# metalcycling/polynomial_reduction_with_full_domain_decomposition_preconditioner

Hardware: AMD Instinct MI355X
Metric: PCG DOF-updates/sec + SpMV GB/s (%HBM peak), 3D Poisson N=7 (higher is better)
Workload: dtype f64; 1 GPU; 3D Poisson, 32x32x32 elements (32^3 per GPU), N=7, flexible PCG + FDD preconditioner (single subdomain = whole domain, inner GMRES(4), polynomial reduction 6); outer=fcg, mesh=box, poly_degree=7, points_per_gpu=16777216, unique_nodes=11390625, preconditioner=fdd_gmres4, comm=single

## Files before the change

include/fdd_hip.h:

```cpp
#ifndef FDD_HIP_H
#define FDD_HIP_H

#include <stddef.h>

#ifdef __cplusplus
extern "C" {
#endif

#define FDD_ERR_INVALID_ARGUMENT (-1)
#define FDD_ERR_UNSUPPORTED (-2)
#define FDD_ERR_NOT_INITIALIZED (-3)

#define FDD_NUM_GEOM_FACTS 6
#define FDD_REDUCE_MAX_BLOCKS 2048

const char *fdd_version(void);
const char *fdd_last_error(void);
int fdd_device_count(int *count);
int fdd_set_device(int device);
int fdd_get_device(int *device);
int fdd_device_name(char *buf, size_t buf_len);
int fdd_malloc(void **ptr, size_t bytes);
int fdd_free(void *ptr);
int fdd_memcpy_h2d(void *dst, const void *src, size_t bytes, void *stream);
// ... 37 lines not shown

int fdd_dom_stiffness_matrix_1(double *const GDu[3], const double *u, const double *D_hat, const double *const G[FDD_NUM_GEOM_FACTS], int num_points, int poly_degree, int dim, void *stream);
int fdd_dom_stiffness_matrix_2(double *Au, const double *const GDu[3], const double *D_hat, int num_points, int poly_degree, int dim, void *stream);
int fdd_dom_stiffness_matrix(double *Au, const double *u, const double *D_hat, const double *const G[FDD_NUM_GEOM_FACTS], int num_elements, int poly_degree, void *stream);

int fdd_stiffness_matrix_mfma(double *Au, const double *u, const double *D_hat, const double *const G[FDD_NUM_GEOM_FACTS], const int *elem_offset, int num_elements, int poly_degree, void *stream);
int fdd_stiffness_matrix_mfma_gather(double *Au, const double *v, const double *v_scale_dev, const int *point_dof, const double *D_hat, const double *const G[FDD_NUM_GEOM_FACTS], const int *elem_offset, int num_elements, int poly_degree, void *stream);
int fdd_stiffness_matrix_mfma_diag(double *Au, const double *v, const double *v_scale_dev, const int *point_dof, const double *D_hat, const double *const G[FDD_NUM_GEOM_FACTS], const int *elem_offset, int num_elements, int poly_degree, void *stream);

int fdd_dom_initialize_arrays(double *u_k, double *r_k, const double *f, int num_points, void *stream);

size_t fdd_reduce_workspace_doubles(void);
int fdd_dom_residual_norm(double *out, double *ws, const double *r_k, const double *QQt_r_k, const double *dirichlet_mask, int num_points, void *stream);
int fdd_dom_projection_inner_products(double *out2, double *ws, const double *z_k, const double *r_k, const double *p_k, const double *q_k, int num_points, void *stream);
int fdd_dom_inner_product_flexible(double *out, double *ws, const double *r_k, const double *r_kp1, const double *z_k, int num_points, void *stream);
int fdd_dom_inner_product_flexible_gamma(double *out2, double *ws, const double *r_k, const double *r_kp1, const double *z_k, int num_points, void *stream);
int fdd_dom_lincomb_flexible_gamma(double *out2, double *ws, const double *r_k, const double *r_kp1, double *z_k, int num_points, int slice_begin, int slice_size, int z_is_zero, const double *coeffs_dev, const double *const *v, const double *v_scale_dev, const double *last_dev, int m, void *stream);
int fdd_dom_inner_product(double *out, double *ws, const double *u_k, const double *v_k, const double *dirichlet_mask, int num_points, void *stream);

int fdd_dom_solution_and_residual_update(double *u_k, double *r_kp1, const double *r_k, const double *p_k, const double *q_k, double alpha_k, int num_points, void *stream);
int fdd_dom_residual_and_search_update(double *p_k, double *r_k, const double *z_k, const double *r_kp1, double beta_k, int num_points, void *stream);
int fdd_dom_solution_and_residual_update_dev(double *u_k, double *r_kp1, const double *r_k, const double *p_k, const double *q_k, const double *alpha_num, const double *alpha_den, int num_points, void *stream);
int fdd_dom_residual_and_search_update_dev(double *p_k, double *r_k, const double *z_k, const double *r_kp1, const double *beta_num, const double *beta_den, int num_points, void *stream);

int fdd_sub_stiffness_matrix_1(double *const GDu[3], const double *u, const double *const *D_hat_ptr, const int *offset, const int *vert, const int *level, const int *poly_degree, int num_levels, const double *const G[FDD_NUM_GEOM_FACTS], int num_points, int dim, void *stream);
int fdd_sub_stiffness_matrix_2(double *Au, const double *const GDu[3], const double *const *D_hat_ptr, const int *offset, const int *vert, const int *level, const int *poly_degree, int num_levels, int num_points, int dim, void *stream);
int fdd_sub_stiffness_matrix(double *Au, const double *u, const double *D_hat, const double *const G[FDD_NUM_GEOM_FACTS], const int *elem_offset, int num_elements, int poly_degree, void *stream);
int fdd_stiffness_matrix_2d(double *Au, const double *u, const double *D_hat, const double *const G[FDD_NUM_GEOM_FACTS], const int *elem_offset, int num_elements, int poly_degree, void *stream);
int fdd_sub_stiffness_matrix_gather(double *Au, const double *v, const int *point_dof, const double *D_hat, const double *const G[FDD_NUM_GEOM_FACTS], const int *elem_offset, int num_elements, int poly_degree, void *stream);

int fdd_sub_inner_product(double *out, double *ws, const double *u, const double *v, int num_values, void *stream);
int fdd_sub_weighted_inner_product(double *out, double *ws, const double *u, const double *v, const double *w, int num_values, void *stream);
int fdd_sub_projection_inner_products(double *out2, double *ws, const double *z_k, const double *r_k, const double *p_k, const double *q_k, const double *weight, int num_values, void *stream);
int fdd_sub_search_update_inner_product(double *out, double *ws, const double *r_k, const double *r_kp1, const double *z_k, const double *weight, int num_points, void *stream);
int fdd_sub_initialize_arrays(double *u_k, double *r_k, const double *f, int num_values, void *stream);
int fdd_sub_solution_and_residual_update(double *u_k, double *r_kp1, const double *r_k, const double *p_k, const double *q_k, double alpha_k, int num_values, void *stream);
int fdd_sub_residual_and_search_update(double *p_k, double *r_k, const double *z_k, const double *r_kp1, double beta_k, int num_values, void *stream);
int fdd_sub_copy_f64_f64(double *u, const double *v, int num_points, void *stream);
int fdd_sub_copy_f32_f64(float *u, const double *v, int num_points, void *stream);
int fdd_sub_copy_f64_f32(double *u, const float *v, int num_points, void *stream);
int fdd_sub_restriction_1(double *Ju, const double *J_cf, const double *u, int num_points, int n_f, int n_c, int dim, void *stream);
int fdd_sub_restriction_2(double *Ju, const double *J_cf, const double *u, int num_points, int n_f, int n_c, int dim, void *stream);
int fdd_sub_restriction_3(double *Ju, const double *J_cf, const double *u, int num_points, int n_f, int n_c, void *stream);
int fdd_sub_restriction(double *u_c, const double *J_cf, const double *u_f, int num_elements, int n_f, int n_c, void *stream);
int fdd_sub_restriction_2d(double *u_c, const double *J_cf, const double *u_f, int num_elements, int n_f, int n_c, void *stream);

// ... 139 lines not shown
```

polynomial_reduction_with_full_domain_decomposition_preconditioner_amd/csrc/fdd_blas1.hip:

```cpp
#include "fdd_stream.h"

namespace
{

constexpr int kBlock = 256;
using Single = fdd_lanes<1>;
using Pair = fdd_lanes<2>;

template <typename Op>
__global__ __launch_bounds__(kBlock) void ew_vec2_kernel(Op op, long long n2, long long n)
{
    const long long stride = (long long)gridDim.x * kBlock;
    for (long long i = (long long)blockIdx.x * kBlock + threadIdx.x; i < n2; i += stride) op.at(Pair{}, i);
    if ((n & 1) && blockIdx.x == 0 && threadIdx.x == 0) op.at(Single{}, n - 1);
}

template <typename Op>
__global__ __launch_bounds__(kBlock) void ew_scalar_kernel(Op op, long long n)
{
    const long long stride = (long long)gridDim.x * kBlock;
    for (long long i = (long long)blockIdx.x * kBlock + threadIdx.x; i < n; i += stride) op.at(Single{}, i);
}

constexpr int kEwMaxBlocks = 32768;
// ... 85 lines not shown
    }
    template <typename F>
    void pointers(F f) const { f(z), f(u), f(d); }
};

struct XpbyRatioDevOp
{
    double *out;
    const double *x, *y, *num, *den;
    template <typename A>
    __device__ void at(A a, long long i) const { a.st(out, i, a.ld(x, i) + (*num / *den) * a.ld(y, i)); }
    template <typename F>
    void pointers(F f) const { f(out), f(x), f(y); }
};

struct XmayRatioDevOp
{
    double *out;
    const double *x, *y, *num, *den;
    template <typename A>
    __device__ void at(A a, long long i) const { a.st(out, i, a.ld(x, i) - (*num / *den) * a.ld(y, i)); }
    template <typename F>
    void pointers(F f) const { f(out), f(x), f(y); }
};

struct ChebyStepOp
{
    double *x, *d, *r_out;
    const double *r_in, *q, *dinv;
    double c_d, c_r;
    int first, last;
    template <typename A>
    __device__ void at(A a, long long i) const { fdd_cheby_step_at(a, i, x, d, r_out, r_in, q, dinv, c_d, c_r, first, last); }
    template <typename F>
    void pointers(F f) const
    {
        f(x), f(r_in), f(dinv);
        if (!last) f(d);
        if (!first) f(q), f(d);
        if (!first && !last) f(r_out);
    }
};

}
__global__ void fdd_sqrt_sum_kernel(double *out, const double *parts, int nparts)
{
// ... 344 lines not shown
{
    FDD_REQUIRE(out != nullptr && parts_dev != nullptr && nparts >= 1);
    hipLaunchKernelGGL(fdd_sqrt_sum_kernel, dim3(1), dim3(64), 0, fdd_stream(stream), out, parts_dev, nparts);
    FDD_LAUNCH_CHECK();
    return 0;
}

int fdd_xpby_ratio_dev(double *out, const double *x, const double *num_dev, const double *den_dev, const double *y, int n, void *stream)
{
    FDD_REQUIRE(n >= 0);
    if (n == 0) return 0;
    FDD_REQUIRE(out != nullptr && x != nullptr && y != nullptr && num_dev != nullptr && den_dev != nullptr);
    return launch_ew(XpbyRatioDevOp{out, x, y, num_dev, den_dev}, n, stream);
}

int fdd_xmay_ratio_dev(double *out, const double *x, const double *num_dev, const double *den_dev, const double *y, int n, void *stream)
{
    FDD_REQUIRE(n >= 0);
    if (n == 0) return 0;
    FDD_REQUIRE(out != nullptr && x != nullptr && y != nullptr && num_dev != nullptr && den_dev != nullptr);
    return launch_ew(XmayRatioDevOp{out, x, y, num_dev, den_dev}, n, stream);
}

int fdd_vector_scaling_dev(double *au, const double *scale_dev, const double *u, int n, void *stream)
{
    FDD_REQUIRE(n >= 0);
    if (n == 0) return 0;
    FDD_REQUIRE(au != nullptr && u != nullptr && scale_dev != nullptr);
    return launch_ew(ScaleDevOp{au, u, scale_dev}, n, stream);
}

int fdd_vector_diagonal_scaling_dev(double *z, const double *d, const double *scale_dev, const double *u, int n, void *stream)
{
    FDD_REQUIRE(n >= 0);
    if (n == 0) return 0;
    FDD_REQUIRE(z != nullptr && u != nullptr && d != nullptr);
    return launch_ew(DiagScaleDevOp{z, d, u, scale_dev}, n, stream);
}

int fdd_cheby_step(double *x, double *d, double *r_out, const double *r_in, const double *q, const double *dinv, double c_d, double c_r, int first, int last, int n, void *stream)
{
    FDD_REQUIRE(n >= 0);
    if (n == 0) return 0;
    FDD_REQUIRE(x != nullptr && r_in != nullptr && dinv != nullptr);
    FDD_REQUIRE(last || d != nullptr);
    FDD_REQUIRE(first || (q != nullptr && d != nullptr && (last || r_out != nullptr)));
// ... 194 lines not shown
```

polynomial_reduction_with_full_domain_decomposition_preconditioner_amd/csrc/fdd_reduce.hip:

```cpp
#include "fdd_stream.h"

namespace
{

constexpr int kBlock = 256;
constexpr int kWaves = kBlock / FDD_WAVE;
using Single = fdd_lanes<1>;
using Pair = fdd_lanes<2>;

template <int NV>
struct Acc
{
    double v[NV];
};

template <int NV>
__device__ __forceinline__ void block_reduce_store(Acc<NV> a, double *ws, int nblocks_stride)
{
    __shared__ double s[NV][kWaves];
    const int lane = threadIdx.x & (FDD_WAVE - 1);
    const int wave = threadIdx.x / FDD_WAVE;

#pragma unroll
    for (int k = 0; k < NV; k++)
// ... 351 lines not shown
    }
    template <typename F>
    void pointers(F f) const
    {
        f(y), f(w), f(dst);
        for (int k = 0; k < M; k++) f(x[k]);
    }
};

template <int M>
int launch_multi_axpy_norm(double *out, double *ws, double *dst, const double *y, const double *c, double sign, const double *const *x, const double *x_scale_dev, const double *w, int n, void *stream)
{
    MultiAxpyNormOp<M> op;
    op.dst = dst;
    op.y = y;
    op.w = w;
    op.c = c;
    op.xs = x_scale_dev;
    op.sign = sign;
    for (int k = 0; k < M; k++) op.x[k] = x[k];
    return launch_reduce(op, out, ws, n, stream);
}

__global__ __launch_bounds__(kBlock) void gather_norm2_kernel(double *ws, const int *__restrict__ Qt_ptr, const int *__restrict__ Qt_col, const double *__restrict__ u, const double *__restrict__ w, int n)
{
    Acc<1> a;
    a.v[0] = 0.0;
    constexpr int NPT = 4;
    const int stride = gridDim.x * kBlock * NPT;
    for (int tile = blockIdx.x * kBlock * NPT; tile < n; tile += stride)
    {
        int j0[NPT], j1[NPT];
        double wn[NPT], s[NPT];
#pragma unroll
        for (int r = 0; r < NPT; r++)
        {
            const int node = tile + r * kBlock + threadIdx.x;
            const bool on = node < n;
            j0[r] = on ? Qt_ptr[node] : 0;
            j1[r] = on ? Qt_ptr[node + 1] : 0;
            wn[r] = on ? w[node] : 0.0;
        }
        fdd_multi_row_sum<NPT, 4, true>(Qt_col, nullptr, u, j0, j1, s);
#pragma unroll
        for (int r = 0; r < NPT; r++)
        {
// ... 129 lines not shown
    return launch_reduce(FlexGammaOp{r_k, r_kp1, z_k}, out2, ws, num_points, stream);
}

int fdd_dom_lincomb_flexible_gamma(double *out2, double *ws, const double *r_k, const double *r_kp1, double *z_k, int num_points, int slice_begin, int slice_size, int z_is_zero, const double *coeffs_dev, const double *const *v, const double *v_scale_dev, const double *last_dev, int m, void *stream)
{
    FDD_REQUIRE(out2 != nullptr && ws != nullptr && num_points >= 0 && m >= 1 && m <= FDD_MULTI_MAX);
    FDD_REQUIRE(slice_begin >= 0 && slice_size >= 0 && (long long)slice_begin + slice_size <= num_points);
    FDD_REQUIRE(num_points == 0 || (r_k != nullptr && r_kp1 != nullptr && z_k != nullptr));
    FDD_REQUIRE(slice_size == 0 || (coeffs_dev != nullptr && v != nullptr));
    if (slice_size == 0) return launch_reduce(FlexGammaOp{r_k, r_kp1, z_k}, out2, ws, num_points, stream);
    for (int k = 0; k < m; k++) FDD_REQUIRE(v[k] != nullptr && v[k] != z_k + slice_begin);
    const bool zero = z_is_zero != 0;
    switch (m)
    {
    case 1: return launch_lincomb_flex_gamma<1>(out2, ws, r_k, r_kp1, z_k, num_points, slice_begin, slice_size, zero, coeffs_dev, v, v_scale_dev, last_dev, stream);
    case 2: return launch_lincomb_flex_gamma<2>(out2, ws, r_k, r_kp1, z_k, num_points, slice_begin, slice_size, zero, coeffs_dev, v, v_scale_dev, last_dev, stream);
    case 3: return launch_lincomb_flex_gamma<3>(out2, ws, r_k, r_kp1, z_k, num_points, slice_begin, slice_size, zero, coeffs_dev, v, v_scale_dev, last_dev, stream);
    case 4: return launch_lincomb_flex_gamma<4>(out2, ws, r_k, r_kp1, z_k, num_points, slice_begin, slice_size, zero, coeffs_dev, v, v_scale_dev, last_dev, stream);
    case 5: return launch_lincomb_flex_gamma<5>(out2, ws, r_k, r_kp1, z_k, num_points, slice_begin, slice_size, zero, coeffs_dev, v, v_scale_dev, last_dev, stream);
    case 6: return launch_lincomb_flex_gamma<6>(out2, ws, r_k, r_kp1, z_k, num_points, slice_begin, slice_size, zero, coeffs_dev, v, v_scale_dev, last_dev, stream);
    case 7: return launch_lincomb_flex_gamma<7>(out2, ws, r_k, r_kp1, z_k, num_points, slice_begin, slice_size, zero, coeffs_dev, v, v_scale_dev, last_dev, stream);
    default: return launch_lincomb_flex_gamma<8>(out2, ws, r_k, r_kp1, z_k, num_points, slice_begin, slice_size, zero, coeffs_dev, v, v_scale_dev, last_dev, stream);
    }
}

int fdd_sub_inner_product(double *out, double *ws, const double *u, const double *v, int num_values, void *stream)
{
    FDD_REQUIRE(out != nullptr && ws != nullptr && num_values >= 0);
    FDD_REQUIRE(num_values == 0 || (u != nullptr && v != nullptr));
    return launch_reduce(Dot2Op{u, v}, out, ws, num_values, stream);
}

int fdd_sub_weighted_inner_product(double *out, double *ws, const double *u, const double *v, const double *w, int num_values, void *stream)
{
    FDD_REQUIRE(out != nullptr && ws != nullptr && num_values >= 0);
    FDD_REQUIRE(num_values == 0 || (u != nullptr && v != nullptr && w != nullptr));
    return launch_reduce(Dot3Op{u, v, w}, out, ws, num_values, stream);
}

int fdd_sub_projection_inner_products(double *out2, double *ws, const double *z_k, const double *r_k, const double *p_k, const double *q_k, const double *weight, int num_values, void *stream)
{
    FDD_REQUIRE(out2 != nullptr && ws != nullptr && num_values >= 0);
    FDD_REQUIRE(num_values == 0 || (z_k != nullptr && r_k != nullptr && p_k != nullptr && q_k != nullptr && weight != nullptr));
    return launch_reduce(ProjWOp{z_k, r_k, p_k, q_k, weight}, out2, ws, num_values, stream);
}

// ... 109 lines not shown
```

polynomial_reduction_with_full_domain_decomposition_preconditioner_amd/host/domain.hpp:

```cpp
#ifndef FDD_DOMAIN_HPP
#define FDD_DOMAIN_HPP

#include <cmath>
#include <cstring>
#include <limits>
#include <string>
#include <unordered_map>
#include <vector>

#include "config.hpp"
#include "csr_matrix.hpp"
#include "element.hpp"
#include "element_operator.hpp"
#include "field_ops.hpp"
#include "gll.hpp"
#include "gmres.hpp"
#include "math.hpp"
#include "projection.hpp"
#include "timer.hpp"

namespace fdd
{
struct PendingUpdate
{
// ... 75 lines not shown
    int va_valid = 0;
    fdd::GmresScalars<DType> gmres_scalars;
    int gmres_point_vectors = 0;

    static constexpr int SLOT_GAMMA = 0;
    static constexpr int SLOT_PQ = 1;
    static constexpr int SLOT_PAIR_A = 2;
    static constexpr int SLOT_THETA = 3;
    static constexpr int SLOT_NORM = 4;
    static constexpr int SLOT_PAIR_B = 6;
    static_assert(SLOT_PAIR_A + 2 == SLOT_NORM and SLOT_NORM + 2 == SLOT_PAIR_B, "a pair and the norm's parts are four contiguous doubles on either side");
    static_assert(SLOT_THETA + 1 == SLOT_NORM and SLOT_THETA == SLOT_PAIR_A + 1, "theta sits right in front of the norm's parts");

    struct FcgRun
    {
        fdd::memory u, u_pts;
        bool nodes_active = false;
        DType r_0_norm = 0.0, gamma_k = 0.0;
        int iter = 0;
        bool norm_pending = false;
        const double *pending_rhs_norm2 = nullptr;
        bool gamma_on_device = false;
        int gamma_slot = SLOT_GAMMA;
    };
    FcgRun fcg;

    struct NormInFlight
    {
        int parts = 1;
        bool deferred = false;
        bool reduce_pending = false;
        const double *source = nullptr;
    };
    NormInFlight norm_state;

    bool nodes_ready = false;
    fdd::memory norm_hist;
    int norm_hist_cap = 0;
    fdd::memory nprefix;
    fdd::memory point_node_dev;
    fdd::memory node_mask;
    fdd::memory node_stitch;
    std::vector<DType> node_stitch_hst, node_mask_hst;
    bool norm_on_dof_slice = false;
    bool stitch_is_one = false;
    fdd::memory node_of_dof, dof_of_node;
// ... 270 lines not shown
    int num_local_points = 0;
    int num_local_nodes = 0;

    int num_elem_points = 0;

    MeshData<DType> mesh;
    std::vector<Element<DType>> elements;

    int num_blocks = 0;
    int num_iterations = 0;
    int num_vectors = 20;
    int max_iterations = 500;
    int preconditioner_type = 1;
    bool use_preconditioner = true;
    bool fused_dssum = true;
    bool neighbour_interface_exchange = true;
    bool restructured_outer = true;
    bool assembled_outer = true;
    bool device_scalars = true;
    bool lazy_steps = true;
    bool shared_residual_norm = true;
    bool early_gamma = true;
    bool fused_update_flexible_dot = true;
    bool unit_stitch_in_place = true;
    fdd::StiffnessFlags stiffness;
    DType tolerance = 1.0e-07;
    std::vector<DType> residual_history;

    fdd::memory D_hat;
    std::vector<double> D_hat_hst;
    fdd::memory geom_fact[NUM_GEOM_FACTS];
    fdd::FieldGeometry field_geometry;

    Domain() {}
    Domain(char *directory_, int poly_degree_) { initialize(directory_, poly_degree_); }
    ~Domain() {}

    int boundary_nodes_count() const { return num_bdary_nodes; }
    int interface_slots_count() const { return num_interface_slots; }
    void comm_probe_interface(int vectors, bool neighbours)
    {
        if (fdd::comm().size == 1 or num_interface_slots == 0) return;
        if (neighbours)
            iface_exchange(vectors == 2 ? 2 : 1);
        else
            fdd::comm().allreduce_sum(interface_slots.as<double>(), (size_t)num_interface_slots * (vectors == 2 ? 2 : 1));
// ... 403 lines not shown
        stitch_is_one = dof_shift >= 0 and not composite_precond and (int)node_stitch_hst.size() >= dof_shift + nd;
        for (int d = 0; d < nd and stitch_is_one; d++)
            if (node_stitch_hst[(size_t)dof_shift + d] != (DType)1.0) stitch_is_one = false;
    }

    void gather_nodes(fdd::memory &t, fdd::memory &v)
    {
        Qt.gather_scatter(nullptr, t.as<double>(), v.as<double>(), nullptr, nullptr, 0, num_local_nodes, 1);
    }

    const fdd::LevelList &operator_list() const { return list; }
    fdd::StiffnessChoice operator_choice() const { return fdd::choose_stiffness(list, stiffness, false, fdd::StiffnessForm::gather); }
    bool set_affine_geometry(bool on)
    {
        list.affine = on and fdd::detect_affine(list);
        return list.affine or not on;
    }

    void stiffness_from_nodes(fdd::memory &q, fdd::memory &pn)
    {
        fdd::apply_gather(list, q.as<double>(), pn.as<double>(), point_node_dev.as<int>(), nullptr, num_local_nodes, stiffness);
    }

    const double *node_norm_enqueue(fdd::memory &rn, bool defer_exchange = false)
    {
        const int nn = num_local_nodes;
        const bool multi = fdd::comm().size > 1 and num_interface_slots > 0;
        const int nb = multi ? num_bdary_nodes : 0;
        double *out = scalars.as<double>() + SLOT_NORM;
        if (multi)
        {
            if (not nprefix.ptr()) nprefix = fdd::dev().malloc<DType>(std::max(num_bdary_nodes, 1));
            nprefix.copyFrom(rn, (size_t)nb * sizeof(DType));
            FDD_CALL(fdd_dom_residual_norm(out + 1, reduce_ws.as<double>(), rn.as<double>() + nb, rn.as<double>() + nb, node_mask.as<double>() + nb, nn - nb, fdd::dev().stream));
            norm_state.parts = 2;
            norm_state.source = rn.as<double>();
            if (defer_exchange)
            {
                norm_state.deferred = true;
                return nullptr;
            }
            gs_add_boundary(nprefix);
            node_norm_finish();
            return nullptr;
        }
        const double *known = nullptr;
        if (norm_on_dof_slice and shared_residual_norm and use_preconditioner)
        {
            const double *self[1] = {rn.as<double>() + dof_shift};
            FDD_CALL(fdd_multi_weighted_inner_product_scaled(out, reduce_ws.as<double>(), self[0], self, nullptr, 1, nullptr, nodes_sub_dofs, fdd::dev().stream));
            known = out;
        }
        else
        {
            const double *self[1] = {rn.as<double>()};
            FDD_CALL(fdd_multi_weighted_inner_product(out, reduce_ws.as<double>(), rn.as<double>(), self, 1, node_mask.as<double>(), nn, fdd::dev().stream));
        }
        norm_state.parts = 1;
        if (fdd::comm().size > 1) fdd::comm().allreduce_sum(out, norm_state.parts);
        return known;
    }

    void node_norm_finish()
    {
        double *out = scalars.as<double>() + SLOT_NORM;
        FDD_CALL(fdd_dom_residual_norm(out, reduce_ws.as<double>(), norm_state.source, nprefix.as<double>(), node_mask.as<double>(), num_bdary_nodes, fdd::dev().stream));
        if (norm_state.deferred and device_scalars)
            norm_state.reduce_pending = true;
        else
            fdd::comm().allreduce_sum(out, 2);
        norm_state.deferred = false;
    }

    DType node_norm_fetch()
    {
        DType v[2] = {0.0, 0.0};
        fdd::memory tail = scalars.slice(SLOT_NORM, 2);
        tail.copyTo(v, norm_state.parts * sizeof(DType));
        return std::sqrt(v[0] + v[1]);
    }

    const double *node_norm(DType &r_norm, fdd::memory &rn)
    {
// ... 74 lines not shown
        if (use_preconditioner) setup_dof_maps(subdomain);
        fcg.u_pts = u;
        fcg.nodes_active = true;

        gather_nodes(nr, f);
        if (use_preconditioner and composite_precond) rp.copyFrom(f, (size_t)num_local_points * sizeof(DType));
        FDD_CALL(fdd_set_to_value(nu.as<double>(), 0.0, num_local_nodes, 0, fdd::dev().stream));
        FDD_CALL(fdd_set_to_value(nz.as<double>(), 0.0, num_local_nodes, 0, fdd::dev().stream));

        const double *r0_norm2 = node_norm(fcg.r_0_norm, nr);
        residual_history.push_back(fcg.r_0_norm);
        rstdout("Iter %2d: | residual_norm = %24.16g | relative_residual_norm = %24.16g | \n", 0, fcg.r_0_norm, 1.0);

        precondition_nodes(nz, nr, subdomain, {r0_norm2});
        np.copyFrom(nz, (size_t)num_local_nodes * sizeof(DType));
    }

    DType fcg_nodes_step_residual()
    {
        const int nn = num_local_nodes;
        void *stream = fdd::dev().stream;
        DType values[2], r_norm;

        fdd_timer().start("domain.operator_application");
        stiffness_from_nodes(q_k, np);
        gather_nodes(nq, q_k);
        fdd_timer().stop("domain.operator_application");

        if (device_scalars and fcg.gamma_on_device and early_gamma)
        {
            FDD_CALL(fdd_sub_inner_product(scalars.as<double>() + SLOT_PQ, reduce_ws.as<double>(), np.as<double>(), nq.as<double>(), nn, stream));
            if (fdd::comm().size > 1) fdd::comm().allreduce_sum(scalars.as<double>() + SLOT_PQ, 1);
        }
        else
        {
            FDD_CALL(fdd_dom_projection_inner_products(scalars.as<double>(), reduce_ws.as<double>(), nz.as<double>(), nr.as<double>(), np.as<double>(), nq.as<double>(), nn, stream));
            if (device_scalars and fdd::comm().size > 1) fdd::comm().allreduce_sum(scalars.as<double>(), 2);
        }
        if (device_scalars)
        {
            if (not(fcg.gamma_on_device and early_gamma)) fcg.gamma_slot = 0;
            FDD_CALL(fdd_dom_solution_and_residual_update_dev(nu.as<double>(), nr1.as<double>(), nr.as<double>(), np.as<double>(), nq.as<double>(), scalars.as<double>() + fcg.gamma_slot, scalars.as<double>() + SLOT_PQ, nn, stream));
            if (use_preconditioner and composite_precond)
                FDD_CALL(fdd_xmay_ratio_dev(rp.as<double>(), rp.as<double>(), scalars.as<double>() + fcg.gamma_slot, scalars.as<double>() + SLOT_PQ, q_k.as<double>(), num_local_points, stream));
            fcg.pending_rhs_norm2 = node_norm_enqueue(nr1, true);
            fcg.norm_pending = true;
            return std::numeric_limits<DType>::quiet_NaN();
        }
        fetch_scalars(values, 2);
        fcg.gamma_k = values[0];
        const DType alpha_k = fcg.gamma_k / values[1];

        FDD_CALL(fdd_dom_solution_and_residual_update(nu.as<double>(), nr1.as<double>(), nr.as<double>(), np.as<double>(), nq.as<double>(), alpha_k, nn, stream));
        if (use_preconditioner and composite_precond) FDD_CALL(fdd_vector_vector_addition(rp.as<double>(), 1.0, rp.as<double>(), -alpha_k, q_k.as<double>(), num_local_points, stream));

        fcg.pending_rhs_norm2 = node_norm(r_norm, nr1);
        residual_history.push_back(r_norm);
        rstdout("Iter %2d: | residual_norm = %24.16g | relative_residual_norm = %24.16g | \n", fcg.iter + 1, r_norm, r_norm / fcg.r_0_norm);
        return r_norm;
    }

    DType fcg_nodes_norm()
    {
        const DType r_norm = node_norm_fetch();
        fcg.norm_pending = false;
        residual_history.push_back(r_norm);
        rstdout("Iter %2d: | residual_norm = %24.16g | relative_residual_norm = %24.16g | \n", fcg.iter + 1, r_norm, r_norm / fcg.r_0_norm);
        return r_norm;
// ... 18 lines not shown
                if (pu.active)
                {
                    pu.active = false;
                    if (pu.q != nz.as<double>() + dof_shift or pu.n > nodes_sub_dofs)
                    {
                        fprintf(stderr, "ERROR: the inner solve's deferred update is not the one of z~'s dof slice\n");
                        exit(EXIT_FAILURE);
                    }
                    const bool rhs_shared = pu.v[0] == nr1.as<double>() + dof_shift;
                    fdd::ProfileScope prof("reduce_vec2_kernel<LincombFlexGamma>", 8.0 * (2.0 * nn + (nn - pu.n) + (double)pu.n * ((double)pu.v.size() + (rhs_shared ? 0 : 1))));
                    FDD_CALL(fdd_dom_lincomb_flexible_gamma(scalars.as<double>() + next, reduce_ws.as<double>(), nr.as<double>(), nr1.as<double>(), nz.as<double>(), nn, dof_shift, pu.n, pu.q_is_zero, pu.coeffs_dev, pu.v.data(),
                                                            pu.scales_dev, pu.last_dev, (int)pu.v.size(), fdd::dev().stream));
                }
                else
                    FDD_CALL(fdd_dom_inner_product_flexible_gamma(scalars.as<double>() + next, reduce_ws.as<double>(), nr.as<double>(), nr1.as<double>(), nz.as<double>(), nn, fdd::dev().stream));
                if (fdd::comm().size > 1)
                {
                    if (norm_state.reduce_pending)
                        fdd::comm().allreduce_sum(scalars.as<double>() + std::min(next, SLOT_NORM), 4);
                    else
                        fdd::comm().allreduce_sum(scalars.as<double>() + next, 2);
                }
                norm_state.reduce_pending = false;
                FDD_CALL(fdd_xpby_ratio_dev(np.as<double>(), nz.as<double>(), scalars.as<double>() + theta_at, scalars.as<double>() + fcg.gamma_slot, np.as<double>(), nn, fdd::dev().stream));
                fcg.gamma_slot = next;
            }
            else
            {
                FDD_CALL(fdd_dom_inner_product_flexible(scalars.as<double>() + SLOT_THETA, reduce_ws.as<double>(), nr.as<double>(), nr1.as<double>(), nz.as<double>(), nn, fdd::dev().stream));
                if (fdd::comm().size > 1) fdd::comm().allreduce_sum(scalars.as<double>() + SLOT_THETA, norm_state.reduce_pending ? 3 : 1);
                norm_state.reduce_pending = false;
                FDD_CALL(fdd_xpby_ratio_dev(np.as<double>(), nz.as<double>(), scalars.as<double>() + SLOT_THETA, scalars.as<double>() + fcg.gamma_slot, np.as<double>(), nn, fdd::dev().stream));
            }
            fcg.gamma_on_device = early_gamma;
            std::swap(nr, nr1);
        }
        else
        {
            fcg.gamma_on_device = false;
            FDD_CALL(fdd_dom_inner_product_flexible(scalars.as<double>(), reduce_ws.as<double>(), nr.as<double>(), nr1.as<double>(), nz.as<double>(), nn, fdd::dev().stream));
            fetch_scalars(&theta_k, 1);
            const DType beta_k = theta_k / fcg.gamma_k;
            FDD_CALL(fdd_dom_residual_and_search_update(np.as<double>(), nr.as<double>(), nz.as<double>(), nr1.as<double>(), beta_k, nn, fdd::dev().stream));
        }
        if (pu.active)
        {
            fprintf(stderr, "ERROR: an inner solve's deferred final update was dropped\n");
            exit(EXIT_FAILURE);
        }
        num_iterations++;
        fcg.iter++;
    }

    void fcg_finish()
    {
        if (not fcg.nodes_active) return;
        Q.multiply(fcg.u_pts, nu);
    }

    template <typename PType>
    void fcg_begin(fdd::memory &u, fdd::memory &f, PType &subdomain)
    {
        residual_history.clear();
        num_iterations = 0;
        fcg = FcgRun();
        norm_state = NormInFlight();
        if (can_fcg_nodes(subdomain))
        {
            fcg_nodes_begin(u, f, subdomain);
            return;
        }
        fcg.u = u;

        fdd_timer().start("domain.vector_operations");
        FDD_CALL(fdd_dom_initialize_arrays(u.as<double>(), r_k.as<double>(), f.as<double>(), num_local_points, fdd::dev().stream));
        fdd_timer().stop("domain.vector_operations");

        fdd_timer().start("domain.residual_norm");
        residual_norm(fcg.r_0_norm, r_k);
// ... 184 lines not shown
                for (auto &v : VP) v = fdd::dev().malloc<DType>(std::max(num_local_points, 1));
            }
            gmres_nodes_vectors = m;
        }
        residual_history.clear();
        norm_state = NormInFlight();

        auto assembled = [&](int i) -> fdd::memory & {
            if (not multi) return VN[i];
            VNA[i].copyFrom(VN[i], (size_t)nn * sizeof(DType));
            gs_add_boundary(VNA[i]);
            return VNA[i];
        };
        auto norm_of = [&](fdd::memory &v) {
            DType norm;
            fdd_timer().start("domain.residual_norm");
            node_norm(norm, v);
            fdd_timer().stop("domain.residual_norm");
            return norm;
        };

        fdd_timer().start("domain.vector_operations");
        gather_nodes(nf, f);
        FDD_CALL(fdd_set_to_value(nu.as<double>(), 0.0, nn, 0, stream));
        nr.copyFrom(nf, (size_t)nn * sizeof(DType));
        if (points_too) VP[0].copyFrom(f, (size_t)num_local_points * sizeof(DType));
        fdd_timer().stop("domain.vector_operations");

        std::vector<const double *> va(m + 1, nullptr);
        std::vector<DType> minus_h(m);
        fdd::GmresSpace<DType> space;
        space.initial_norm = [&] { return norm_of(nr); };
        space.restart_norm = [&] {
            fdd_timer().start("domain.operator_application");
            stiffness_from_nodes(q_k, nu);
            gather_nodes(nq, q_k);
            fdd_timer().stop("domain.operator_application");
            fdd_timer().start("domain.vector_operations");
            FDD_CALL(fdd_vector_vector_addition(nr.as<double>(), 1.0, nf.as<double>(), -1.0, nq.as<double>(), nn, stream));
            if (points_too) FDD_CALL(fdd_vector_vector_addition(VP[0].as<double>(), 1.0, f.as<double>(), -1.0, q_k.as<double>(), num_local_points, stream));
            fdd_timer().stop("domain.vector_operations");
            return norm_of(nr);
        };
        space.start_cycle = [&](DType gamma_0) {
            fdd_timer().start("domain.vector_operations");
            FDD_CALL(fdd_vector_scaling(VN[0].as<double>(), 1.0 / gamma_0, nr.as<double>(), nn, stream));
// ... 256 lines not shown
```

polynomial_reduction_with_full_domain_decomposition_preconditioner_amd/host/fdd_device.hpp:

```cpp
#ifndef FDD_DEVICE_HPP
#define FDD_DEVICE_HPP

#include <cstddef>
#include <cstdio>
#include <cstdlib>
#include <string>
#include <utility>
#include <vector>

#include "fdd_hip.h"

#pragma weak fdd_amg_setup_row_pointers
#pragma weak fdd_amg_setup_spgemm_count
#pragma weak fdd_amg_setup_spgemm_fill
#pragma weak fdd_amg_setup_transpose_count
#pragma weak fdd_amg_setup_transpose_fill
#pragma weak fdd_amg_setup_fem_stencils
#pragma weak fdd_amg_setup_fem_count
#pragma weak fdd_amg_setup_fem_fill
#pragma weak fdd_amg_setup_inv_sqrt_diagonal
#pragma weak fdd_amg_setup_unit_values
#pragma weak fdd_amg_setup_lattice_dofs
#pragma weak fdd_amg_setup_lattice_coarse_flags
#pragma weak fdd_amg_setup_lattice_cmap
#pragma weak fdd_amg_setup_lattice_interp_count
#pragma weak fdd_amg_setup_lattice_interp_fill
#pragma weak fdd_amg_setup_lattice_coarse_points
#pragma weak fdd_amg_setup_memory_info
#pragma weak fdd_dom_lincomb_flexible_gamma
#pragma weak fdd_projection_dots
#pragma weak fdd_projection_apply
#pragma weak fdd_projection_store
#pragma weak fdd_cheby_step
#pragma weak fdd_cheby_step_f32
#pragma weak fdd_csr_plan_gather_cheby
#pragma weak fdd_csr_plan_gather_cheby_f32
#pragma weak fdd_stiffness_matrix_diag
#pragma weak fdd_stiffness_matrix_diag_f32
#pragma weak fdd_stiffness_offdiag_zero
#pragma weak fdd_stiffness_matrix_mfma_diag
#pragma weak fdd_stiffness_matrix_lines
#pragma weak fdd_stiffness_matrix_lines_f32
#pragma weak fdd_stiffness_matrix_lines_shared
#pragma weak fdd_stiffness_matrix_lines_shared_f32
#pragma weak fdd_stiffness_factor_block_hash
#pragma weak fdd_stiffness_factor_block_verify
#pragma weak fdd_stiffness_matrix_lines_lean
#pragma weak fdd_stiffness_matrix_lines_lean_f32
#pragma weak fdd_stiffness_matrix_lines_direct
#pragma weak fdd_csr_plan_gather_mapped
#pragma weak fdd_field_mass
#pragma weak fdd_field_gradient
// ... 230 lines not shown
```

polynomial_reduction_with_full_domain_decomposition_preconditioner_amd/host/fdd_host_capi.cpp:

```cpp
#include "fdd_host.h"

#include <atomic>
#include <chrono>
#include <cmath>
#include <cstdarg>
#include <cstring>
#include <limits>
#include <exception>
#include <memory>
#include <string>
#include <sys/stat.h>
#include <unordered_map>
#include <functional>
#include <vector>

#include "box_mesh.hpp"
#include "domain.hpp"
#include "field_ops.hpp"
#include "subdomain.hpp"

typedef double SType;
typedef double PType;

static thread_local char g_err[512] = "";
// ... 912 lines not shown

struct PlainFlagRow
{
    const char *name;
    bool Domain<SType>::*domain;
    bool Subdomain<PType>::*subdomain;
};

static const PlainFlagRow *plain_flag_row(const std::string &flag)
{
    typedef Domain<SType> D;
    typedef Subdomain<PType> S;
    static const PlainFlagRow table[] = {
        {"fused_dssum", &D::fused_dssum, &S::fused_dssum},
        {"restructured_inner_solve", &D::restructured_outer, &S::restructured},
        {"neighbour_interface_exchange", &D::neighbour_interface_exchange, nullptr},
        {"fold_coarse_exchange", nullptr, &S::fold_coarse_exchange},
        {"assembled_outer_solve", &D::assembled_outer, nullptr},
        {"shared_residual_norm", &D::shared_residual_norm, nullptr},
        {"skip_last_basis_store", nullptr, &S::skip_last_basis_store},
        {"early_gamma", &D::early_gamma, nullptr},
        {"unit_stitch_in_place", &D::unit_stitch_in_place, nullptr},
        {"fused_update_flexible_dot", &D::fused_update_flexible_dot, nullptr},
        {"lazy_steps", &D::lazy_steps, nullptr},
        {"device_bookkeeping", &D::device_scalars, &S::device_bookkeeping},
        {"assembled_inner_solve", nullptr, &S::assembled_inner},
    };
    for (const PlainFlagRow &row : table)
        if (flag == row.name) return &row;
    return nullptr;
}

static int set_amg_device_setup(fddh_problem &p, const char *, int value)
{
    if (value != 0)
        if (const char *missing = fdd::missing_amg_setup_entry()) return fail("amg_device_setup needs %s, which the loaded kernel library does not export", missing);
    p.subdomain->amg_device_setup = value != 0;
    return 0;
}

static int set_sub_use_preconditioner(fddh_problem &p, const char *, int value)
{
    p.subdomain->use_preconditioner = value == 1;
    p.subdomain->use_jacobi = value == 2;
    return 0;
}
// ... 779 lines not shown
```

Before: 8.779 billion DOF-updates/s.

## Fuse residual update with norm and defer solution update into direction pass

The outer flexible CG step now fuses the residual update r1 = r - alpha*q with the squared-norm reduction into one kernel, so r1 is no longer read back for a separate norm. The solution update u += alpha*p is deferred and merged into the later direction update p = z + beta*p, which already reads p, saving a pass over p. Deferred updates are flushed before operator application, at the end of the solve, and on non-device paths. This adds bookkeeping state and two more kernels, and the fused norm only applies when the norm is a single-slice sum.

```diff
diff --git a/include/fdd_hip.h b/include/fdd_hip.h
--- a/include/fdd_hip.h
+++ b/include/fdd_hip.h
@@ -83,6 +83,8 @@
 int fdd_dom_residual_and_search_update(double *p_k, double *r_k, const double *z_k, const double *r_kp1, double beta_k, int num_points, void *stream);
 int fdd_dom_solution_and_residual_update_dev(double *u_k, double *r_kp1, const double *r_k, const double *p_k, const double *q_k, const double *alpha_num, const double *alpha_den, int num_points, void *stream);
 int fdd_dom_residual_and_search_update_dev(double *p_k, double *r_k, const double *z_k, const double *r_kp1, const double *beta_num, const double *beta_den, int num_points, void *stream);
+int fdd_dom_residual_update_norm2_dev(double *out, double *ws, double *r_kp1, const double *r_k, const double *q_k, const double *alpha_num, const double *alpha_den, int num_points, int slice_begin, int slice_size, void *stream);
+int fdd_dom_solution_direction_update_dev(double *u_k, double *p_k, const double *z_k, const double *alpha_num, const double *alpha_den, const double *beta_num, const double *beta_den, int num_points, void *stream);
 
 int fdd_sub_stiffness_matrix_1(double *const GDu[3], const double *u, const double *const *D_hat_ptr, const int *offset, const int *vert, const int *level, const int *poly_degree, int num_levels, const double *const G[FDD_NUM_GEOM_FACTS], int num_points, int dim, void *stream);
 int fdd_sub_stiffness_matrix_2(double *Au, const double *const GDu[3], const double *const *D_hat_ptr, const int *offset, const int *vert, const int *level, const int *poly_degree, int num_levels, int num_points, int dim, void *stream);
diff --git a/polynomial_reduction_with_full_domain_decomposition_preconditioner_amd/csrc/fdd_blas1.hip b/polynomial_reduction_with_full_domain_decomposition_preconditioner_amd/csrc/fdd_blas1.hip
--- a/polynomial_reduction_with_full_domain_decomposition_preconditioner_amd/csrc/fdd_blas1.hip
+++ b/polynomial_reduction_with_full_domain_decomposition_preconditioner_amd/csrc/fdd_blas1.hip
@@ -131,6 +131,22 @@
     __device__ void at(A a, long long i) const { a.st(out, i, a.ld(x, i) - (*num / *den) * a.ld(y, i)); }
     template <typename F>
     void pointers(F f) const { f(out), f(x), f(y); }
+};
+
+struct SolutionDirectionDevOp
+{
+    double *u, *p;
+    const double *z, *a_num, *a_den, *b_num, *b_den;
+    template <typename A>
+    __device__ void at(A a, long long i) const
+    {
+        const double al = a_num[0] / a_den[0];
+        const auto uu = a.ld(u, i), pp = a.ld(p, i), zz = a.ld(z, i);
+        a.st(u, i, uu + al * pp);
+        a.st(p, i, zz + (*b_num / *b_den) * pp);
+    }
+    template <typename F>
+    void pointers(F f) const { f(u), f(p), f(z); }
 };
 
 struct ChebyStepOp
@@ -521,6 +537,14 @@
     return launch_ew(XmayRatioDevOp{out, x, y, num_dev, den_dev}, n, stream);
 }
 
+int fdd_dom_solution_direction_update_dev(double *u_k, double *p_k, const double *z_k, const double *alpha_num, const double *alpha_den, const double *beta_num, const double *beta_den, int num_points, void *stream)
+{
+    FDD_REQUIRE(num_points >= 0);
+    if (num_points == 0) return 0;
+    FDD_REQUIRE(u_k != nullptr && p_k != nullptr && z_k != nullptr && u_k != p_k && alpha_num != nullptr && alpha_den != nullptr && beta_num != nullptr && beta_den != nullptr);
+    return launch_ew(SolutionDirectionDevOp{u_k, p_k, z_k, alpha_num, alpha_den, beta_num, beta_den}, num_points, stream);
+}
+
 int fdd_vector_scaling_dev(double *au, const double *scale_dev, const double *u, int n, void *stream)
 {
     FDD_REQUIRE(n >= 0);
diff --git a/polynomial_reduction_with_full_domain_decomposition_preconditioner_amd/csrc/fdd_reduce.hip b/polynomial_reduction_with_full_domain_decomposition_preconditioner_amd/csrc/fdd_reduce.hip
--- a/polynomial_reduction_with_full_domain_decomposition_preconditioner_amd/csrc/fdd_reduce.hip
+++ b/polynomial_reduction_with_full_domain_decomposition_preconditioner_amd/csrc/fdd_reduce.hip
@@ -397,6 +397,56 @@
     return launch_reduce(op, out, ws, n, stream);
 }
 
+struct ResidualUpdateNormOp
+{
+    double *r1;
+    const double *r, *q, *num, *den;
+    template <typename A>
+    __device__ typename A::template value<double> at(A l, long long from, long long i, bool wide_loads = true) const
+    {
+        const double al = num[0] / den[0];
+        typename A::template value<double> rr, qq;
+        if constexpr (std::is_same<A, Pair>::value)
+        {
+            if (wide_loads)
+                rr = l.ld(r + from, i), qq = l.ld(q + from, i);
+            else
+            {
+                rr = {__builtin_nontemporal_load(r + from + 2 * i), __builtin_nontemporal_load(r + from + 2 * i + 1)};
+                qq = {__builtin_nontemporal_load(q + from + 2 * i), __builtin_nontemporal_load(q + from + 2 * i + 1)};
+            }
+        }
+        else
+            rr = l.ld(r + from, i), qq = l.ld(q + from, i);
+        const auto v = rr - al * qq;
+        l.st(r1 + from, i, v);
+        return v;
+    }
+    template <typename A, typename V>
+    static __device__ __forceinline__ void add(A l, Acc<1> &acc, V v) { l.add(acc.v[0], v * v * l.all(1.0)); }
+};
+
+template <bool PAIRS>
+__global__ __launch_bounds__(kBlock) void residual_update_norm_kernel(ResidualUpdateNormOp op, double *ws, long long lo, long long nd, long long n, bool wide_loads)
+{
+    Acc<1> a;
+    a.v[0] = 0.0;
+    const long long stride = (long long)gridDim.x * kBlock;
+    const long long first = (long long)blockIdx.x * kBlock + threadIdx.x;
+    if constexpr (PAIRS)
+    {
+        const long long nd2 = nd / 2;
+        for (long long i = first; i < nd2; i += stride) ResidualUpdateNormOp::add(Pair{}, a, op.at(Pair{}, lo, i, wide_loads));
+        if ((nd & 1) && first == 0) ResidualUpdateNormOp::add(Single{}, a, op.at(Single{}, lo, nd - 1));
+    }
+    else
+        for (long long i = first; i < nd; i += stride) ResidualUpdateNormOp::add(Single{}, a, op.at(Single{}, lo, i));
+    for (long long i = first; i < lo; i += stride) op.at(Single{}, 0, i);
+    for (long long i = lo + nd + first; i < n; i += stride) op.at(Single{}, 0, i);
+
+    block_reduce_store<1>(a, ws, FDD_REDUCE_MAX_BLOCKS);
+}
+
 __global__ __launch_bounds__(kBlock) void gather_norm2_kernel(double *ws, const int *__restrict__ Qt_ptr, const int *__restrict__ Qt_col, const double *__restrict__ u, const double *__restrict__ w, int n)
 {
     Acc<1> a;
@@ -572,6 +622,35 @@
     case 7: return launch_lincomb_flex_gamma<7>(out2, ws, r_k, r_kp1, z_k, num_points, slice_begin, slice_size, zero, coeffs_dev, v, v_scale_dev, last_dev, stream);
     default: return launch_lincomb_flex_gamma<8>(out2, ws, r_k, r_kp1, z_k, num_points, slice_begin, slice_size, zero, coeffs_dev, v, v_scale_dev, last_dev, stream);
     }
+}
+
+int fdd_dom_residual_update_norm2_dev(double *out, double *ws, double *r_kp1, const double *r_k, const double *q_k, const double *alpha_num, const double *alpha_den, int num_points, int slice_begin, int slice_size, void *stream)
+{
+    FDD_REQUIRE(out != nullptr && ws != nullptr && num_points >= 0);
+    FDD_REQUIRE(slice_begin >= 0 && slice_size >= 0 && (long long)slice_begin + slice_size <= num_points);
+    FDD_REQUIRE(num_points == 0 || (r_kp1 != nullptr && r_k != nullptr && q_k != nullptr && alpha_num != nullptr && alpha_den != nullptr));
+    hipStream_t s = fdd_stream(stream);
+    const ResidualUpdateNormOp op{r_kp1, r_k, q_k, alpha_num, alpha_den};
+    const long long lo = slice_begin, nd = slice_size, n = num_points;
+    const bool pairs = nd >= 2 && fdd_aligned(r_kp1 + lo, Pair::bytes<double>);
+    const bool wide_loads = fdd_aligned(r_k + lo, Pair::bytes<double>) && fdd_aligned(q_k + lo, Pair::bytes<double>);
+    if (nd == 0)
+    {
+        if (hipError_t e = hipMemsetAsync(out, 0, sizeof(double), s)) return (int)e;
+        if (n == 0) return 0;
+        hipLaunchKernelGGL(residual_update_norm_kernel<false>, dim3(fdd_stream_grid(n, kBlock)), dim3(kBlock), 0, s, op, ws, lo, nd, n, wide_loads);
+        FDD_LAUNCH_CHECK();
+        return 0;
+    }
+    const int grid = fdd_stream_grid(pairs ? nd / 2 : nd, kBlock);
+    if (pairs)
+        hipLaunchKernelGGL(residual_update_norm_kernel<true>, dim3(grid), dim3(kBlock), 0, s, op, ws, lo, nd, n, wide_loads);
+    else
+        hipLaunchKernelGGL(residual_update_norm_kernel<false>, dim3(grid), dim3(kBlock), 0, s, op, ws, lo, nd, n, wide_loads);
+    FDD_LAUNCH_CHECK();
+    hipLaunchKernelGGL(reduce_final_kernel<1>, dim3(1), dim3(kBlock), 0, s, out, ws, grid);
+    FDD_LAUNCH_CHECK();
+    return 0;
 }
 
 int fdd_sub_inner_product(double *out, double *ws, const double *u, const double *v, int num_values, void *stream)
diff --git a/polynomial_reduction_with_full_domain_decomposition_preconditioner_amd/host/domain.hpp b/polynomial_reduction_with_full_domain_decomposition_preconditioner_amd/host/domain.hpp
--- a/polynomial_reduction_with_full_domain_decomposition_preconditioner_amd/host/domain.hpp
+++ b/polynomial_reduction_with_full_domain_decomposition_preconditioner_amd/host/domain.hpp
@@ -121,6 +121,12 @@
         const double *pending_rhs_norm2 = nullptr;
         bool gamma_on_device = false;
         int gamma_slot = SLOT_GAMMA;
+        struct OwedSolutionUpdate
+        {
+            bool active = false;
+            const double *num = nullptr, *den = nullptr;
+        };
+        OwedSolutionUpdate owed_u;
     };
     FcgRun fcg;
 
@@ -437,6 +443,8 @@
     bool shared_residual_norm = true;
     bool early_gamma = true;
     bool fused_update_flexible_dot = true;
+    bool fused_residual_norm = true;
+    bool solution_in_direction_pass = true;
     bool unit_stitch_in_place = true;
     fdd::StiffnessFlags stiffness;
     DType tolerance = 1.0e-07;
@@ -886,6 +894,12 @@
         fdd::apply_gather(list, q.as<double>(), pn.as<double>(), point_node_dev.as<int>(), nullptr, num_local_nodes, stiffness);
     }
 
+    bool norm_is_slice_sum() const
+    {
+        const bool multi = fdd::comm().size > 1 and num_interface_slots > 0;
+        return not multi and norm_on_dof_slice and shared_residual_norm and use_preconditioner;
+    }
+
     const double *node_norm_enqueue(fdd::memory &rn, bool defer_exchange = false)
     {
         const int nn = num_local_nodes;
@@ -909,7 +923,7 @@
             return nullptr;
         }
         const double *known = nullptr;
-        if (norm_on_dof_slice and shared_residual_norm and use_preconditioner)
+        if (norm_is_slice_sum())
         {
             const double *self[1] = {rn.as<double>() + dof_shift};
             FDD_CALL(fdd_multi_weighted_inner_product_scaled(out, reduce_ws.as<double>(), self[0], self, nullptr, 1, nullptr, nodes_sub_dofs, fdd::dev().stream));
@@ -923,6 +937,16 @@
         norm_state.parts = 1;
         if (fdd::comm().size > 1) fdd::comm().allreduce_sum(out, norm_state.parts);
         return known;
+    }
+
+    const double *residual_update_and_norm_enqueue(fdd::memory &rn1, fdd::memory &rn, fdd::memory &qn, const double *num, const double *den)
+    {
+        const int nn = num_local_nodes;
+        double *out = scalars.as<double>() + SLOT_NORM;
+        fdd::ProfileScope prof("residual_update_norm_kernel", 24.0 * nn);
+        FDD_CALL(fdd_dom_residual_update_norm2_dev(out, reduce_ws.as<double>(), rn1.as<double>(), rn.as<double>(), qn.as<double>(), num, den, nn, dof_shift, nodes_sub_dofs, fdd::dev().stream));
+        norm_state.parts = 1;
+        return out;
     }
 
     void node_norm_finish()
@@ -1043,6 +1067,8 @@
         void *stream = fdd::dev().stream;
         DType values[2], r_norm;
 
+        fcg_flush_solution_update();
+
         fdd_timer().start("domain.operator_application");
         stiffness_from_nodes(q_k, np);
         gather_nodes(nq, q_k);
@@ -1061,10 +1087,25 @@
         if (device_scalars)
         {
             if (not(fcg.gamma_on_device and early_gamma)) fcg.gamma_slot = 0;
-            FDD_CALL(fdd_dom_solution_and_residual_update_dev(nu.as<double>(), nr1.as<double>(), nr.as<double>(), np.as<double>(), nq.as<double>(), scalars.as<double>() + fcg.gamma_slot, scalars.as<double>() + SLOT_PQ, nn, stream));
+            const double *a_num = scalars.as<double>() + fcg.gamma_slot, *a_den = scalars.as<double>() + SLOT_PQ;
+            const bool defer_u = solution_in_direction_pass and &fdd_dom_solution_direction_update_dev != nullptr;
+            const bool fuse_norm = fused_residual_norm and &fdd_dom_residual_update_norm2_dev != nullptr and norm_is_slice_sum();
+            if (not defer_u and not fuse_norm)
+                FDD_CALL(fdd_dom_solution_and_residual_update_dev(nu.as<double>(), nr1.as<double>(), nr.as<double>(), np.as<double>(), nq.as<double>(), a_num, a_den, nn, stream));
+            else
+            {
+                if (defer_u)
+                    fcg.owed_u = {true, a_num, a_den};
+                else
+                    FDD_CALL(fdd_xpby_ratio_dev(nu.as<double>(), nu.as<double>(), a_num, a_den, np.as<double>(), nn, stream));
+                if (fuse_norm)
+                    fcg.pending_rhs_norm2 = residual_update_and_norm_enqueue(nr1, nr, nq, a_num, a_den);
+                else
+                    FDD_CALL(fdd_xmay_ratio_dev(nr1.as<double>(), nr.as<double>(), a_num, a_den, nq.as<double>(), nn, stream));
+            }
             if (use_preconditioner and composite_precond)
-                FDD_CALL(fdd_xmay_ratio_dev(rp.as<double>(), rp.as<double>(), scalars.as<double>() + fcg.gamma_slot, scalars.as<double>() + SLOT_PQ, q_k.as<double>(), num_local_points, stream));
-            fcg.pending_rhs_norm2 = node_norm_enqueue(nr1, true);
+                FDD_CALL(fdd_xmay_ratio_dev(rp.as<double>(), rp.as<double>(), a_num, a_den, q_k.as<double>(), num_local_points, stream));
+            if (not fuse_norm) fcg.pending_rhs_norm2 = node_norm_enqueue(nr1, true);
             fcg.norm_pending = true;
             return std::numeric_limits<DType>::quiet_NaN();
         }
@@ -1129,7 +1170,7 @@
                         fdd::comm().allreduce_sum(scalars.as<double>() + next, 2);
                 }
                 norm_state.reduce_pending = false;
-                FDD_CALL(fdd_xpby_ratio_dev(np.as<double>(), nz.as<double>(), scalars.as<double>() + theta_at, scalars.as<double>() + fcg.gamma_slot, np.as<double>(), nn, fdd::dev().stream));
+                direction_update_dev(scalars.as<double>() + theta_at, scalars.as<double>() + fcg.gamma_slot);
                 fcg.gamma_slot = next;
             }
             else
@@ -1137,7 +1178,7 @@
                 FDD_CALL(fdd_dom_inner_product_flexible(scalars.as<double>() + SLOT_THETA, reduce_ws.as<double>(), nr.as<double>(), nr1.as<double>(), nz.as<double>(), nn, fdd::dev().stream));
                 if (fdd::comm().size > 1) fdd::comm().allreduce_sum(scalars.as<double>() + SLOT_THETA, norm_state.reduce_pending ? 3 : 1);
                 norm_state.reduce_pending = false;
-                FDD_CALL(fdd_xpby_ratio_dev(np.as<double>(), nz.as<double>(), scalars.as<double>() + SLOT_THETA, scalars.as<double>() + fcg.gamma_slot, np.as<double>(), nn, fdd::dev().stream));
+                direction_update_dev(scalars.as<double>() + SLOT_THETA, scalars.as<double>() + fcg.gamma_slot);
             }
             fcg.gamma_on_device = early_gamma;
             std::swap(nr, nr1);
@@ -1145,6 +1186,7 @@
         else
         {
             fcg.gamma_on_device = false;
+            fcg_flush_solution_update();
             FDD_CALL(fdd_dom_inner_product_flexible(scalars.as<double>(), reduce_ws.as<double>(), nr.as<double>(), nr1.as<double>(), nz.as<double>(), nn, fdd::dev().stream));
             fetch_scalars(&theta_k, 1);
             const DType beta_k = theta_k / fcg.gamma_k;
@@ -1159,9 +1201,30 @@
         fcg.iter++;
     }
 
+    void direction_update_dev(const double *b_num, const double *b_den)
+    {
+        const int nn = num_local_nodes;
+        if (fcg.owed_u.active)
+        {
+            fdd::ProfileScope prof("ew_kernel<SolutionDirectionDev>", 40.0 * nn);
+            FDD_CALL(fdd_dom_solution_direction_update_dev(nu.as<double>(), np.as<double>(), nz.as<double>(), fcg.owed_u.num, fcg.owed_u.den, b_num, b_den, nn, fdd::dev().stream));
+            fcg.owed_u.active = false;
+        }
+        else
+            FDD_CALL(fdd_xpby_ratio_dev(np.as<double>(), nz.as<double>(), b_num, b_den, np.as<double>(), nn, fdd::dev().stream));
+    }
+
+    void fcg_flush_solution_update()
+    {
+        if (not fcg.owed_u.active) return;
+        FDD_CALL(fdd_xpby_ratio_dev(nu.as<double>(), nu.as<double>(), fcg.owed_u.num, fcg.owed_u.den, np.as<double>(), num_local_nodes, fdd::dev().stream));
+        fcg.owed_u.active = false;
+    }
+
     void fcg_finish()
     {
         if (not fcg.nodes_active) return;
+        fcg_flush_solution_update();
         Q.multiply(fcg.u_pts, nu);
     }
 
@@ -1392,6 +1455,7 @@
 
         fdd_timer().start("domain.vector_operations");
         gather_nodes(nf, f);
+        fcg.owed_u.active = false;
         FDD_CALL(fdd_set_to_value(nu.as<double>(), 0.0, nn, 0, stream));
         nr.copyFrom(nf, (size_t)nn * sizeof(DType));
         if (points_too) VP[0].copyFrom(f, (size_t)num_local_points * sizeof(DType));
diff --git a/polynomial_reduction_with_full_domain_decomposition_preconditioner_amd/host/fdd_device.hpp b/polynomial_reduction_with_full_domain_decomposition_preconditioner_amd/host/fdd_device.hpp
--- a/polynomial_reduction_with_full_domain_decomposition_preconditioner_amd/host/fdd_device.hpp
+++ b/polynomial_reduction_with_full_domain_decomposition_preconditioner_amd/host/fdd_device.hpp
@@ -28,6 +28,8 @@
 #pragma weak fdd_amg_setup_lattice_coarse_points
 #pragma weak fdd_amg_setup_memory_info
 #pragma weak fdd_dom_lincomb_flexible_gamma
+#pragma weak fdd_dom_residual_update_norm2_dev
+#pragma weak fdd_dom_solution_direction_update_dev
 #pragma weak fdd_projection_dots
 #pragma weak fdd_projection_apply
 #pragma weak fdd_projection_store
diff --git a/polynomial_reduction_with_full_domain_decomposition_preconditioner_amd/host/fdd_host_capi.cpp b/polynomial_reduction_with_full_domain_decomposition_preconditioner_amd/host/fdd_host_capi.cpp
--- a/polynomial_reduction_with_full_domain_decomposition_preconditioner_amd/host/fdd_host_capi.cpp
+++ b/polynomial_reduction_with_full_domain_decomposition_preconditioner_amd/host/fdd_host_capi.cpp
@@ -958,6 +958,8 @@
         {"early_gamma", &D::early_gamma, nullptr},
         {"unit_stitch_in_place", &D::unit_stitch_in_place, nullptr},
         {"fused_update_flexible_dot", &D::fused_update_flexible_dot, nullptr},
+        {"fused_residual_norm", &D::fused_residual_norm, nullptr},
+        {"solution_in_direction_pass", &D::solution_in_direction_pass, nullptr},
         {"lazy_steps", &D::lazy_steps, nullptr},
         {"device_bookkeeping", &D::device_scalars, &S::device_bookkeeping},
         {"assembled_inner_solve", nullptr, &S::assembled_inner},
```

Result: faster. 9.006 billion DOF-updates/s (median of 6 runs) (+2.6%).
